# SamsungLabs/cloud_transformers

Measured on AMD Instinct MI355X. Metric: points/sec fwd+bwd MHCT, 4096-pt batch, 1/2/4/8 MI355X; % HBM roofline, higher is better.
Workload: dtype f32; 1 GPU; north-star op-level: B=8 clouds x N=4096 pts, H=64 heads, C=16 feat/head, 2D grid W=32, reduce=max, keys=tanh(randn), seed 1234+rank; step = Splat fwd, Slice fwd, Slice bwd, Splat bwd (key cotangents summed); per_gpu_batch=8, parallelism=replica-sharded clouds x1 (no collective), world_size_seen=1, hip_graph=True, steps_per_graph=10

## Files before the change

cloud_transformers_amd/_lib.py:

```python
import ctypes
import os
import subprocess
import threading

import torch

_HERE = os.path.dirname(os.path.abspath(__file__))
CSRC = os.path.join(_HERE, "csrc")
LIB_DIR = os.path.join(_HERE, "lib")
LIB_PATH = os.environ.get("CLOUDCT_LIB") or os.path.join(LIB_DIR, "libcloudct.so")
INCLUDE = os.path.join(os.path.dirname(_HERE), "include")

HIP_SOURCES = ["ct_raster.hip", "ct_mhct.hip", "ct_lattice.hip", "ct_gconv.hip", "ct_chamfer.hip", "ct_emd.hip",
               "ct_adain.hip", "ct_bnorm.hip", "ct_pwgemm.hip", "ct_nbr.hip", "ct_kpitems.hip", "ct_completion.hip", "ct_scanitems.hip",
               "ct_blockitems.hip", "ct_kpplan.hip", "ct_imageitems.hip", "ct_voxel.hip"]
HIPCC_FLAGS = ["-O3", "--offload-arch=gfx950", "-std=c++17", "-fPIC", "-shared",
               "-ffp-contract=off"]

class BnFwdItem(ctypes.Structure):
    _fields_ = [("x", ctypes.c_void_p), ("x_batch_stride", ctypes.c_longlong), ("weight", ctypes.c_void_p), ("bias", ctypes.c_void_p),
                ("running_mean", ctypes.c_void_p), ("running_var", ctypes.c_void_p), ("num_batches_tracked", ctypes.c_void_p),
                ("residual", ctypes.c_void_p), ("residual_batch_stride", ctypes.c_longlong), ("y", ctypes.c_void_p),
                ("y_batch_stride", ctypes.c_longlong), ("save_mean", ctypes.c_void_p), ("save_rstd", ctypes.c_void_p),
                ("amax_out", ctypes.c_void_p), ("C", ctypes.c_int), ("eps", ctypes.c_float), ("momentum", ctypes.c_float),
# ... 155 lines not shown
    deps = srcs + [os.path.join(INCLUDE, "cloudct_host.h")]
    if not force and os.path.exists(HOST_LIB_PATH) and all(os.path.getmtime(d) <= os.path.getmtime(HOST_LIB_PATH) for d in deps):
        return HOST_LIB_PATH
    import fcntl
    os.makedirs(LIB_DIR, exist_ok=True)
    with open(os.path.join(LIB_DIR, ".build_host.lock"), "w") as lock:
        fcntl.flock(lock, fcntl.LOCK_EX)
        try:
            tmp = "%s.%d.tmp" % (HOST_LIB_PATH, os.getpid())
            subprocess.run([os.environ.get("CXX", "g++"), "-O2", "-std=c++17", "-fPIC", "-shared", "-ffp-contract=off", "-I", INCLUDE]
                           + srcs + ["-o", tmp], check=True)
            os.replace(tmp, HOST_LIB_PATH)
        finally:
            fcntl.flock(lock, fcntl.LOCK_UN)
    return HOST_LIB_PATH


def load_host():
    global _host
    if _host is None:
        with _lock:
            if _host is None:
                lib = ctypes.CDLL(build_host())
                f32p, i32p = ctypes.POINTER(ctypes.c_float), ctypes.POINTER(ctypes.c_int32)
                lib.ct_grid_subsample.restype = ctypes.c_int64
                lib.ct_grid_subsample.argtypes = [f32p, f32p, i32p, ctypes.c_int64, ctypes.c_int, ctypes.c_int, ctypes.c_float,
                                                  f32p, f32p, i32p]
                _host = lib
    return _host


_vp, _i, _f, _sz = ctypes.c_void_p, ctypes.c_int, ctypes.c_float, ctypes.c_size_t
_ll = ctypes.c_longlong
_ip = ctypes.POINTER(ctypes.c_int)
_fp = ctypes.POINTER(ctypes.c_float)

SIGNATURES = {
    "ct_abi_version": (_i, []),
    "ct_strerror": (ctypes.c_char_p, [_i]),
    "ct_set_deterministic": (None, [_i]),
    "ct_get_deterministic": (_i, []),
    "ct_deterministic_override": (None, [_i]),
    "ct_positions_fwd": (_i, [_vp, _vp, _vp, _i, _i, _i, _i, _ip, _vp]),
    "ct_positions_bwd": (_i, [_vp, _vp, _vp, _i, _i, _i, _i, _ip, _vp]),
    "ct_splat_fwd": (_i, [_vp, _vp, _vp, _i, _vp, _i, _i, _i, _i, _i, _ip, _i, _vp]),
    "ct_splat_bwd_workspace_bytes": (_sz, [_i, _i, _i, _i, _i, _ip, _i]),
    "ct_splat_bwd": (_i, [_vp, _vp, _vp, _i, _vp, _vp, _vp, _vp, _vp, _sz, _i, _i, _i, _i, _i, _ip, _i, _vp]),
    "ct_splat_bwd_ex_workspace_bytes": (_sz, [_i, _i, _i, _i, _i, _ip, _i, _i]),
    "ct_splat_bwd_ex": (_i, [_vp, _vp, _vp, _i, _vp, _vp, _vp, _vp, _vp, _sz, _i, _i, _i, _i, _i, _ip, _i, _i, _vp]),
    "ct_debug_set_flags": (None, [ctypes.c_uint]),
    "ct_debug_set_nseg": (None, [_i]),
    "ct_debug_last_launch": (ctypes.c_char_p, []),
    "ct_slice_fwd": (_i, [_vp, _vp, _vp, _i, _vp, _i, _i, _i, _i, _i, _ip, _vp]),
    "ct_slice_bwd": (_i, [_vp, _vp, _vp, _i, _vp, _vp, _vp, _i, _i, _i, _i, _i, _ip, _vp]),
    "ct_slice_bwd_workspace_bytes": (_sz, [_i, _i, _i, _i, _i, _ip]),
    "ct_slice_bwd_ws": (_i, [_vp, _vp, _vp, _i, _vp, _vp, _vp, _vp, _sz, _i, _i, _i, _i, _i, _ip, _vp]),
    "ct_tickets_init": (_i, [_vp, _vp]),
    "ct_splat_bwd_tk_segments": (_i, [_i, _i, _i, _i, _i, _ip]),
    "ct_slice_bwd_tk": (_i, [_vp, _vp, _vp, _i, _vp, _vp, _vp, _vp, _sz, _vp, _i, _i, _i, _i, _i, _ip, _vp]),
    "ct_plane_sort_bytes": (_sz, [_i, _i, _i, _i, _ip]),
    "ct_plane_sort": (_i, [_vp, _vp, _sz, _i, _i, _i, _i, _ip, _vp]),
    "ct_slice_bwd_ps": (_i, [_vp, _vp, _vp, _i, _vp, _vp, _vp, _vp, _sz, _vp, _vp, _i, _i, _i, _i, _i, _ip, _vp]),
    "ct_splat_bwd_tk": (_i, [_vp, _vp, _vp, _i, _vp, _vp, _vp, _vp, _vp, _vp, _sz, _vp, _i, _i, _i, _i, _i, _ip, _i, _vp]),
    "ct_slice_bwd_grid": (_i, [_vp, _vp, _i, _vp, _vp, _i, _i, _i, _i, _i, _ip, _vp]),
    "ct_slice_bwd_keys": (_i, [_vp, _vp, _vp, _i, _vp, _vp, _i, _i, _i, _i, _i, _ip, _vp]),
    "ct_splat_lc_fwd": (_i, [_vp, _vp, _vp, _vp, _i, _vp, _i, _i, _i, _i, _i, _ip, _i, _vp]),
    "ct_splat_lc_bwd": (_i, [_vp, _vp, _vp, _vp, _i, _vp, _vp, _vp, _vp, _vp, _sz, _i, _i, _i, _i, _i, _ip, _i, _vp]),
    "ct_slice_lc_fwd": (_i, [_vp, _vp, _vp, _vp, _i, _vp, _i, _i, _i, _i, _i, _ip, _vp]),
    "ct_slice_lc_bwd": (_i, [_vp, _vp, _vp, _vp, _i, _vp, _vp, _vp, _i, _i, _i, _i, _i, _ip, _vp]),
    "ct_grid_occupancy": (_i, [_vp, ctypes.c_int64, _vp, _vp]),
    "ct_grid_occupancy_ratio": (_i, [_vp, ctypes.c_int64, _f, _vp, _vp, _vp]),
    "ct_lattice_fwd_workspace_bytes": (_sz, [_i, _i, _i]),
    "ct_lattice_fwd": (_i, [_vp, _vp, _vp, _vp, _vp, _vp, _vp, _vp, _vp, _vp, _sz, _i, _i, _i, _i, _vp]),
    "ct_lattice_bwd_workspace_bytes": (_sz, [_i, _i, _i]),
    "ct_lattice_bwd": (_i, [_vp] * 15 + [_vp, _sz, _i, _i, _i, _i, _vp]),
    "ct_lattice_so3_fwd": (_i, [_vp, _vp, _vp, _f, _vp, _vp, _vp, _vp, _vp, _vp, _vp, _vp, _sz, _vp, _i, _i, _i, _i, _vp]),
    "ct_lattice_so3_bwd": (_i, [_vp, _vp, _vp, _f] + [_vp] * 14 + [_vp, _sz, _i, _i, _i, _i, _vp]),
    "ct_so3_exp_fwd": (_i, [_vp, _vp, _i, _f, _vp]),
    "ct_so3_exp_bwd": (_i, [_vp, _vp, _vp, _i, _f, _vp]),
    "ct_adain_group_fwd": (_i, [_vp, _i, _i, _i, _vp]),
    "ct_adain_group_bwd": (_i, [_vp, _i, _i, _i, _vp]),
    "ct_bn_relu_supported": (_i, [_i, _i, _i]),
    "ct_bn_group_fwd": (_i, [_vp, _i, _i, _i, _vp]),
    "ct_bn_group_bwd": (_i, [_vp, _i, _i, _i, _vp]),
    "ct_bn_group_stats_fwd": (_i, [_vp, _i, _i, _i, _i, _i, _vp, _vp]),
    "ct_bn_group_apply_fwd": (_i, [_vp, _i, _i, _i, _i, _i, _vp, _i, _vp, _vp]),
    "ct_bn_group_reduce_bwd": (_i, [_vp, _i, _i, _i, _i, _i, _vp, _vp, _vp]),
    "ct_bn_group_apply_bwd": (_i, [_vp, _i, _i, _i, _i, _i, _vp, _vp, _vp]),
    "ct_bn_eval_supported": (_i, [_i, _i, _i]),
    "ct_bn_eval_group_fwd": (_i, [_vp, _i, _i, _i, _vp]),
    "ct_bn_eval_group_bwd": (_i, [_vp, _i, _i, _i, _vp]),
    "ct_gconv_fwd": (_i, [_vp, _vp, _vp, _vp, _i, _i, _i, _i, _i, _ip, _vp]),
    "ct_gconv_fwd_norm_supported": (_i, [_i, _i, _i, _i, _i, _ip]),
    "ct_gconv_fwd_norm": (_i, [_vp, _vp, _vp, _vp, _vp, _vp, _i, _vp, _i, _i, _i, _i, _i, _ip, _vp]),
    "ct_gconv_bwd_data": (_i, [_vp, _vp, _vp, _i, _i, _i, _i, _i, _ip, _vp]),
    "ct_gconv_supported": (_i, [_i, _i, _i, _i, _i, _ip]),
    "ct_set_gconv_precision": (None, [_i]),
    "ct_get_gconv_precision": (_i, []),
    "ct_gconv_precision_override": (None, [_i]),
    "ct_gconv_precision_covers": (_i, [_i, _i, _i, _i, _i, _i, _ip]),
    "ct_gconv_bwd_weight_workspace_bytes": (_sz, [_i, _i, _i, _i, _i, _ip]),
    "ct_gconv_bwd_weight": (_i, [_vp, _vp, _vp, _vp, _vp, _sz, _i, _i, _i, _i, _i, _ip, _vp]),
    "ct_mhct_core_supported": (_i, [_i, _i, _i, _i, _i, _ip]),
    "ct_mhct_core_workspace_bytes": (_sz, [_i, _i, _i, _i, _i, _ip]),
    "ct_mhct_core_workspace_init": (_i, [_vp, _sz, _i, _i, _i, _i, _i, _ip, _vp]),
    "ct_mhct_core_fwd": (_i, [_vp, _vp, _vp, _i, _vp, _vp, _vp, _vp, _vp, _vp, _vp, _sz, _i, _i, _i, _i, _i, _ip, _vp]),
# ... 104 lines not shown
```

cloud_transformers_amd/csrc/ct_raster.hip:

```cpp
#include "ct_common.h"
#include <string.h>
#include <type_traits>
#include <algorithm>
#include <atomic>
#include <mutex>

#ifndef CT_QUAD_THREADS
#define CT_QUAD_THREADS 512
#endif
#ifndef CT_QUAD_WAVES
#define CT_QUAD_WAVES 4
#endif
#ifndef CT_QUAD_CG
#define CT_QUAD_CG 4
#endif

namespace {

#include "ct_raster_args.h"

__device__ __forceinline__ float stats_MK(const RasterArgs& a, size_t bh, int ch, const float* tile, int G) {
  if (a.stats != nullptr) {
    const size_t per = (size_t)a.B * a.H * a.C;
    unsigned m = 0u, k = 0u;
// ... 933 lines not shown
          if (atomic) {
#pragma unroll
            for (int i = 0; i < 4; ++i) atomicAdd(pk + i, gs[i][j]);
          } else {
            float4 o = make_float4(gs[0][j], gs[1][j], gs[2][j], gs[3][j]);
            if (!first || a.accumulate) {
              const float4 prev = *(const float4*)pk;
              o.x += prev.x; o.y += prev.y; o.z += prev.z; o.w += prev.w;
            }
            *(float4*)pk = o;
          }
        }
      }
    }
    if (STATS) {
      __syncthreads();
      for (int ch = threadIdx.x; ch < cc; ch += blockDim.x) {
        unsigned m = 0u;
        for (int j = 0; j < 32; ++j) m = max(m, s_max[ch * 32 + j]);
        s_max[ch * 32] = m;
      }
      __syncthreads();
      unsigned kmax = 0;
      if (first) {
        for (int i = threadIdx.x; i <= a.cnt_mask; i += blockDim.x) kmax = max(kmax, (unsigned)s_cnt[i]);
        for (int o = 32; o > 0; o >>= 1) kmax = max(kmax, (unsigned)__shfl_xor((int)kmax, o, 64));
      }
      unsigned* slots = (unsigned*)(a.tile_out + toff);
      const bool split = a.nsplit > 1;
      unsigned* mine = a.stats != nullptr ? a.stats + ((size_t)sp * a.B * a.H * a.C + bh * a.C) * 2 : nullptr;
      if (first) {
        if ((threadIdx.x & 63) == 0) atomicMax((unsigned*)&s_cnt[0], kmax);
        __syncthreads();
        const unsigned kall = (unsigned)s_cnt[0];
        for (int ch = threadIdx.x; ch < a.C; ch += blockDim.x) {
          unsigned* kslot = (unsigned*)(a.tile_out + (bh * a.C + ch) * (size_t)g.G) + 1;
          if (mine != nullptr) mine[2 * ch + 1] = kall;
          else if (split) atomicAdd(kslot, kall);
          else *kslot = kall;
        }
      }
      for (int ch = threadIdx.x; ch < cc; ch += blockDim.x) {
        if (mine != nullptr) mine[2 * (c0 + ch)] = s_max[ch * 32];
        else if (split) atomicMax(slots + (size_t)ch * g.G, s_max[ch * 32]);
        else slots[(size_t)ch * g.G] = s_max[ch * 32];
      }
    }
    first = false;
  }
  if constexpr (NORM) norm_store_amax(am, lds, a.amax);
}

#include "ct_raster_hot.h"
#include "ct_raster_hot3d.h"
CT_KERNARG_IS_ARGS_AND_GRID((splat_max_bwd_hot_kernel<false, 32, 2>), 2);
CT_KERNARG_IS_ARGS_AND_GRID((splat_max_bwd_hot_kernel<true, 0, 0, kHotWideThreads>), 2);
#include "ct_raster_band.h"
#include "ct_raster_sorted.h"
#include "ct_raster_sorted3d.h"

template <int DIM>
__global__ void positions_fwd_kernel(const float* keys, float* lc, long long* idx, int BH, int N, GridW<DIM> g) {
  constexpr int V = 1 << DIM;
  size_t i = (size_t)blockIdx.x * blockDim.x + threadIdx.x;
  if (i >= (size_t)BH * N) return;
  size_t bh = i / N;
  int n = (int)(i % N);
  float w0[DIM], w1[DIM];
  int f[DIM];
#pragma unroll
  for (int j = 0; j < DIM; ++j) ct_axis(keys[(bh * DIM + j) * N + n], g.hw[j], g.W[j], w0[j], w1[j], f[j]);
  Corners<DIM> c;
  ct_corners<DIM>(w0, w1, f, g, c);
#pragma unroll
  for (int v = 0; v < V; ++v) {
    lc[(bh * V + v) * N + n] = c.w[v];
    idx[(bh * V + v) * N + n] = (long long)c.cell[v];
  }
}

template <int DIM>
__global__ void positions_bwd_kernel(const float* keys, const float* g_lc, float* g_keys, int BH, int N, GridW<DIM> g) {
  constexpr int V = 1 << DIM;
  size_t i = (size_t)blockIdx.x * blockDim.x + threadIdx.x;
  if (i >= (size_t)BH * N) return;
  size_t bh = i / N;
  int n = (int)(i % N);
  float w0[DIM], w1[DIM], mask[DIM], gw[V], gs[DIM];
  int f[DIM];
#pragma unroll
  for (int j = 0; j < DIM; ++j) {
    float k = keys[(bh * DIM + j) * N + n];
    ct_axis(k, g.hw[j], g.W[j], w0[j], w1[j], f[j]);
    mask[j] = ct_key_mask(k);
  }
#pragma unroll
  for (int v = 0; v < V; ++v) gw[v] = g_lc[(bh * V + v) * N + n];
  ct_corner_grad<DIM>(w0, w1, gw, gs);
#pragma unroll
  for (int j = 0; j < DIM; ++j) g_keys[(bh * DIM + j) * N + n] = gs[j] * mask[j];
}

__global__ void __launch_bounds__(1024) occupancy_kernel(const float* grid, long long n, unsigned long long* count) {
  __shared__ unsigned s_part[16];
  unsigned local = 0;
  const long long n4 = n >> 2;
// ... 48 lines not shown
    __hip_atomic_store(ws + 1 + blockIdx.x, t, __ATOMIC_RELAXED, __HIP_MEMORY_SCOPE_AGENT);
    asm volatile("s_waitcnt vmcnt(0)" ::: "memory");
    const unsigned old = __hip_atomic_fetch_add((unsigned*)ws, 1u, __ATOMIC_RELAXED, __HIP_MEMORY_SCOPE_AGENT);
    s_last = old == gridDim.x - 1u;
    if (old == gridDim.x - 1u) {
      __hip_atomic_store((unsigned*)ws, 0u, __ATOMIC_RELAXED, __HIP_MEMORY_SCOPE_AGENT);
      __builtin_amdgcn_fence(__ATOMIC_ACQUIRE, "agent");
      asm volatile("s_waitcnt vmcnt(0)" ::: "memory");
    }
  }
  __syncthreads();
  if (s_last) {
    unsigned long long t = 0;
    for (unsigned i = threadIdx.x; i < gridDim.x; i += blockDim.x)
      t += __hip_atomic_load(ws + 1 + i, __ATOMIC_RELAXED, __HIP_MEMORY_SCOPE_AGENT);
    unsigned lo = (unsigned)t;
    for (int off = 32; off > 0; off >>= 1) lo += __shfl_down(lo, off, 64);
    __syncthreads();
    if ((threadIdx.x & 63) == 0) s_part[threadIdx.x >> 6] = lo;
    __syncthreads();
    if (threadIdx.x == 0) {
      unsigned long long tot = 0;
      for (int w = 0; w < (int)(blockDim.x >> 6); ++w) tot += s_part[w];
      out[0] = (float)(long long)tot * inv;
    }
  }
}

__global__ void zero_slots_kernel(float* tiles, size_t stride, size_t rows) {
  const size_t r = (size_t)blockIdx.x * blockDim.x + threadIdx.x;
  if (r < rows) {
    tiles[r * stride] = 0.0f;
    tiles[r * stride + 1] = 0.0f;
  }
}

std::atomic<unsigned> t_dbg_flags{0};
std::atomic<int> t_dbg_nseg{0};
std::atomic<int> t_deterministic{0};
thread_local int t_det_override = -1;
inline bool det_now() { return t_det_override >= 0 ? t_det_override != 0 : t_deterministic.load(std::memory_order_relaxed) != 0; }
std::mutex t_last_mu;
char t_last[256] = "";

using ct_tags::note;
using ct_tags::note_reset;

struct Switches {
  unsigned flags;
  int nseg;
  int sorted;
  bool wide;
  bool det;
  bool has(unsigned f) const { return (flags & f) != 0; }
  bool hot() const { return !has(CT_DEBUG_NO_HOT); }
};
Switches read_switches() {
  static const auto env = [](const char* name, int unset) {
    const char* e = getenv(name);
    return e ? atoi(e) : unset;
  };
  static const int sorted = env("CLOUDCT_SORTED", -1), wide = env("CLOUDCT_WIDE", 1), nseg = env("CLOUDCT_SPLAT_BWD_NSEG", 0);
  const int dbg = t_dbg_nseg.load(std::memory_order_relaxed);
  return {t_dbg_flags.load(std::memory_order_relaxed), dbg ? dbg : nseg, sorted, wide != 0,
          det_now()};
}

struct Plan {
  int CC, nchunks, threads;
  size_t lds_bytes;
  bool lds_tile;
};

bool valid_common(int B, int H, int C, int N, int dim, const int* W) {
  if (B <= 0 || H <= 0 || C <= 0 || N <= 0 || (dim != 2 && dim != 3) || !W) return false;
  long long G = 1;
  for (int j = 0; j < dim; ++j) {
    if (W[j] < 2) return false;
    G *= W[j];
    if (G > (1ll << 30)) return false;
  }
  if (H > 65535 || B > 65535) return false;
  return true;
}

template <int DIM>
GridW<DIM> make_grid(const int* W) {
  GridW<DIM> g;
  g.G = 1;
  for (int j = 0; j < DIM; ++j) {
    g.W[j] = W[j];
    g.hw[j] = (float)(W[j] - 1) * 0.5f;
    g.G *= W[j];
  }
  return g;
}

int round_threads(int n) {
  int t = ((n + 63) / 64) * 64;
  return t < 64 ? 64 : (t > 1024 ? 1024 : t);
}

Plan make_plan(int B, int H, int C, int N, int G, int tiles_per_wg ,
               long long want = 256 , int min_cc = 4 ) {
  if (min_cc == 4 && (long long)B * H <= 64) min_cc = 1;
  Plan p;
  size_t per_ch = (size_t)G * 4 * tiles_per_wg;
  p.lds_tile = true;
  if (per_ch > (size_t)kBigLdsBytes) {
    p.lds_tile = false;
    p.CC = C;
    p.nchunks = 1;
    p.lds_bytes = 0;
    p.threads = round_threads(N);
    return p;
  }
  int cc_fit = (int)(kMaxLdsBytes / per_ch);
  if (cc_fit < min_cc) cc_fit = (int)((size_t)kBigLdsBytes / per_ch) < min_cc ? (int)((size_t)kBigLdsBytes / per_ch) : min_cc;
// ... 1020 lines not shown
  if (pg.lds_bytes + extra > (size_t)kBigLdsBytes) return CT_EINVAL;
  ga.cnt_mask = cnt - 1;
  ga.CC = pg.CC; ga.nchunks = pg.nchunks; ga.ncg = 1; ga.atomic_gpos = 0;
  ga.nsplit = slice_bwd_stats_nsplit(a.B, a.H, a.N);
  const size_t stats_bytes = (size_t)ga.nsplit * a.B * a.H * a.C * 2 * 4;
  unsigned* stats = nullptr;
  if (ga.nsplit > 1) {
    if (ws != nullptr && ws_bytes >= stats_bytes && ((uintptr_t)ws & 3) == 0) {
      stats = (unsigned*)ws;
    } else {
      const size_t rows = (size_t)a.B * a.H * a.C;
      CT_CLEAR_ERROR();
      hipLaunchKernelGGL(zero_slots_kernel, dim3((unsigned)((rows + 255) / 256)), dim3(256), 0, st, a.tile_out, (size_t)g.G, rows);
      CT_CHECK_LAUNCH();
    }
  }
  ga.stats = stats;
  dim3 ggrid(ga.nsplit, a.H, a.B);
  if (launch_quad<DIM, QM_GATHER_GW, (DIM == 2 ? CT_QUAD_CG : 2), CT_QUAD_THREADS, true>(ggrid, quad_threads(a.N, ga.nsplit), pg.lds_bytes + extra, st,
                                                                                         ga, g) != CT_OK)
    return CT_ELAUNCH;
  RasterArgs sa = a;
  sa.CC = ps.CC; sa.nchunks = ps.nchunks;
  sa.stats = stats; sa.nsplit = ga.nsplit;
  const int sthreads = ps.threads;
  dim3 sgrid(sa.nchunks, a.H, a.B);
  note(ga.nsplit > 1 ? (stats != nullptr ? "slice_bwd_gw_stats_parts" : "slice_bwd_gw_stats_nsplit") : "slice_bwd_gw_stats");
  if (scatter_quad_ok(sa, true, g.G)) {
    const int qt = scatter_quad_threads(DIM, a.N);
    if (sa.pad_dtype != CT_PAD_NONE) CT_LAUNCH((scatter_quad_kernel<DIM, true, true>), sgrid, qt, (size_t)sa.CC * g.G * 4 + (size_t)sa.CC * 8, st, sa, g);
    else CT_LAUNCH((scatter_quad_kernel<DIM, true, false>), sgrid, qt, (size_t)sa.CC * g.G * 4 + (size_t)sa.CC * 8, st, sa, g);
    note("scatter_quad_add");
    return CT_OK;
  }
  CT_LAUNCH((scatter_add_fx_stream_kernel<DIM, true>), sgrid, sthreads, (size_t)sa.CC * g.G * 4 + (size_t)2 * sa.CC * 4, st, sa, g);
  note("scatter_add_fx_stream");
  return CT_OK;
}

bool valid_pad(const void* pad, int pad_dtype) {
  if (pad_dtype == CT_PAD_NONE) return true;
  return (pad_dtype == CT_PAD_F32 || pad_dtype == CT_PAD_I32) && pad != nullptr;
}

RasterArgs base_args(int B, int H, int C, int N, const void* pad, int pad_dtype) {
  RasterArgs a = {};
  a.B = B; a.H = H; a.C = C; a.N = N;
  a.pad = pad_dtype == CT_PAD_NONE ? nullptr : pad;
  a.pad_dtype = pad_dtype;
  a.nsplit = 1; a.ncg = 1; a.nchunks = 1; a.CC = C;
  return a;
}

template <bool FROM_KEYS>
int splat_fwd_impl(PosSrc pos, const float* feat, const void* pad, int pad_dtype, float* grid,
                   int B, int H, int C, int N, int dim, const int* W, int reduce, hipStream_t st) {
  if (!valid_common(B, H, C, N, dim, W) || !feat || !grid || !valid_pad(pad, pad_dtype)) return CT_EINVAL;
  if (reduce != CT_REDUCE_MAX0 && reduce != CT_REDUCE_SUM) return CT_EINVAL;
  note_reset();
  const Switches sw = read_switches();
  RasterArgs a = base_args(B, H, C, N, pad, pad_dtype);
  a.pos = pos; a.src = feat; a.tile_out = grid;
  return dim == 2 ? run_scatter<2, FROM_KEYS>(sw, a, W, reduce == CT_REDUCE_SUM, st)
                  : run_scatter<3, FROM_KEYS>(sw, a, W, reduce == CT_REDUCE_SUM, st);
}

template <bool FROM_KEYS>
int splat_bwd_impl(PosSrc pos, const float* feat, const void* pad, int pad_dtype, const float* grid,
                   const float* g_grid, float* g_feat, float* g_pos, void* ws, size_t ws_bytes,
                   int B, int H, int C, int N, int dim, const int* W, int reduce, hipStream_t st,
                   const float* g_pos_add = nullptr, void* tickets = nullptr, const Switches* outer = nullptr) {
  if (!valid_common(B, H, C, N, dim, W) || !feat || !g_grid || !g_feat || !g_pos || !valid_pad(pad, pad_dtype)) return CT_EINVAL;
  note_reset();
  const Switches sw = outer ? *outer : read_switches();
  if (g_pos_add != nullptr) {
    const bool in_place = g_pos_add == g_pos;
    const size_t gpos_n = (size_t)B * H * (FROM_KEYS ? dim : (1 << dim)) * N;
    if (in_place && (!ws || ws_bytes < gpos_n * 4)) return CT_EWORKSPACE;
    const size_t head = in_place ? ws_bytes - gpos_n * 4 : ws_bytes;
    if (reduce == CT_REDUCE_MAX0 && grid) {
      RasterArgs a = base_args(B, H, C, N, pad, pad_dtype);
      a.pos = pos; a.src = feat; a.dst = g_feat; a.g_pos = g_pos; a.tile_in = grid; a.tile_in2 = g_grid;
      a.accumulate = in_place ? 1 : 0;
      a.gpos_add = g_pos_add;
      a.tickets = (unsigned*)tickets;
      const int r = dim == 2 ? run_splat_max_bwd<2, FROM_KEYS>(sw, a, W, ws, head, st) : run_splat_max_bwd<3, FROM_KEYS>(sw, a, W, ws, head, st);
      if (r != CT_EINVAL) return r;
    }
    if constexpr (FROM_KEYS) {
      if (reduce == CT_REDUCE_SUM && dim == 2) {
        RasterArgs a = base_args(B, H, C, N, pad, pad_dtype);
        a.pos = pos; a.src = feat; a.dst = g_feat; a.g_pos = g_pos; a.tile_in = g_grid;
        a.gpos_add = g_pos_add;
        const int r = run_splat_sum_bwd_hot(sw, a, make_grid<2>(W), st);
        if (r != CT_EINVAL) return r;
      }
    }
    float* tmp = in_place ? (float*)((char*)ws + head) : g_pos;
    const int r = splat_bwd_impl<FROM_KEYS>(pos, feat, pad, pad_dtype, grid, g_grid, g_feat, tmp, ws, head, B, H, C, N, dim, W,
                                            reduce, st, nullptr, tickets, &sw);
    if (r != CT_OK) return r;
    CT_CLEAR_ERROR();
    hipLaunchKernelGGL(add_inplace_kernel, dim3((unsigned)((gpos_n + 255) / 256)), dim3(256), 0, st, g_pos,
                       in_place ? (const float*)tmp : g_pos_add, gpos_n);
    CT_CHECK_LAUNCH();
    note("add_inplace");
// ... 143 lines not shown
  if (!valid_common(B, H, C, N, dim, W) || reduce != CT_REDUCE_MAX0) return 0;
  size_t n = splat_bwd_workspace_generic(B, H, C, N, dim, W);
  if (det_now()) {
    size_t G = 1;
    for (int j = 0; j < dim; ++j) G *= W[j];
    n = std::max(n, splat_bwd_det_plan(B, H, C, N, dim, (int)G).workspace());
  }
  const size_t hot = dim == 2 ? splat_bwd_hot_workspace(B, H, C, N, make_grid<2>(W)) : splat_bwd_hot_workspace(B, H, C, N, make_grid<3>(W));
  return std::max(n, hot);
}

int ct_splat_bwd(const float* keys, const float* feat, const void* pad, int pad_dtype, const float* grid,
                 const float* g_grid, float* g_feat, float* g_keys, void* ws, size_t ws_bytes,
                 int B, int H, int C, int N, int dim, const int* W, int reduce, ct_stream_t s) {
  if (!keys) return CT_EINVAL;
  PosSrc pos = {keys, nullptr, nullptr};
  return splat_bwd_impl<true>(pos, feat, pad, pad_dtype, grid, g_grid, g_feat, g_keys, ws, ws_bytes,
                              B, H, C, N, dim, W, reduce, (hipStream_t)s);
}

size_t ct_splat_bwd_ex_workspace_bytes(int B, int H, int C, int N, int dim, const int* W, int reduce, int flags) {
  size_t n = ct_splat_bwd_workspace_bytes(B, H, C, N, dim, W, reduce);
  if ((flags & CT_BWD_ACCUMULATE_KEYS) && valid_common(B, H, C, N, dim, W)) n += (size_t)B * H * dim * N * 4;
  return n;
}

int ct_splat_bwd_ex(const float* keys, const float* feat, const void* pad, int pad_dtype, const float* grid,
                    const float* g_grid, float* g_feat, float* g_keys, void* ws, size_t ws_bytes,
                    int B, int H, int C, int N, int dim, const int* W, int reduce, int flags, ct_stream_t s) {
  if (!keys || (flags & ~CT_BWD_ACCUMULATE_KEYS)) return CT_EINVAL;
  PosSrc pos = {keys, nullptr, nullptr};
  return splat_bwd_impl<true>(pos, feat, pad, pad_dtype, grid, g_grid, g_feat, g_keys, ws, ws_bytes,
                              B, H, C, N, dim, W, reduce, (hipStream_t)s, (flags & CT_BWD_ACCUMULATE_KEYS) ? g_keys : nullptr);
}

void ct_debug_set_flags(unsigned flags) { t_dbg_flags = flags; }

void ct_set_deterministic(int on) { t_deterministic.store(on ? 1 : 0, std::memory_order_relaxed); }
int ct_get_deterministic(void) { return det_now() ? 1 : 0; }
void ct_deterministic_override(int on) { t_det_override = on < 0 ? -1 : (on ? 1 : 0); }

const char* ct_debug_last_launch(void) {
  static thread_local char copy[256];
  std::lock_guard<std::mutex> lk(t_last_mu);
  memcpy(copy, t_last, sizeof(copy));
  return copy;
}

int ct_slice_fwd(const float* keys, const float* grid, const void* pad, int pad_dtype, float* out,
                 int B, int H, int C, int N, int dim, const int* W, ct_stream_t s) {
  if (!keys) return CT_EINVAL;
  PosSrc pos = {keys, nullptr, nullptr};
  return slice_fwd_impl<true>(pos, grid, pad, pad_dtype, out, B, H, C, N, dim, W, (hipStream_t)s);
}

int ct_slice_bwd(const float* keys, const float* grid, const void* pad, int pad_dtype, const float* g_out,
                 float* g_grid, float* g_keys, int B, int H, int C, int N, int dim, const int* W, ct_stream_t s) {
  if (!keys) return CT_EINVAL;
  PosSrc pos = {keys, nullptr, nullptr};
  return slice_bwd_impl<true>(pos, grid, pad, pad_dtype, g_out, g_grid, g_keys, B, H, C, N, dim, W, (hipStream_t)s);
}

size_t ct_slice_bwd_workspace_bytes(int B, int H, int C, int N, int dim, const int* W) {
  if (!valid_common(B, H, C, N, dim, W)) return 0;
  const Switches sw = read_switches();
  const size_t hot = dim == 2 ? slice_bwd_hot_workspace(sw, B, H, C, N, make_grid<2>(W)) : slice_bwd_hot_workspace(sw, B, H, C, N, make_grid<3>(W));
  const int ns = slice_bwd_stats_nsplit(B, H, N);
  const size_t stats = ns > 1 ? (size_t)ns * B * H * C * 8 : 0;
  return hot > stats ? hot : stats;
}

int ct_slice_bwd_ws(const float* keys, const float* grid, const void* pad, int pad_dtype, const float* g_out,
                    float* g_grid, float* g_keys, void* ws, size_t ws_bytes, int B, int H, int C, int N, int dim,
                    const int* W, ct_stream_t s) {
  if (!keys) return CT_EINVAL;
  PosSrc pos = {keys, nullptr, nullptr};
  return slice_bwd_impl<true>(pos, grid, pad, pad_dtype, g_out, g_grid, g_keys, B, H, C, N, dim, W, (hipStream_t)s, ws, ws_bytes);
}

void ct_debug_set_nseg(int nseg) { t_dbg_nseg.store(nseg, std::memory_order_relaxed); }

int ct_splat_bwd_tk_segments(int B, int H, int C, int N, int dim, const int* W) {
  if (!valid_common(B, H, C, N, dim, W)) return 1;
  const Switches sw = read_switches();
  long long G = 1;
  for (int j = 0; j < dim; ++j) G *= W[j];
  if (!hot_shape_ok(sw, B, H, C, N, (int)G, 0) || (long long)B * H > CT_TICKETS_BYTES / 8) return 1;
  if (sw.det && !sw.has(CT_DEBUG_FORCE_BAND)) return 1;
  if (sw.has(CT_DEBUG_FORCE_BAND) && C == 4 && ((G / W[0]) & 3) == 0 && W[0] >= 4) return 2;
  HotPlan sp;
  const int nseg = splat_bwd_segments_plan(sw, B, H, C, N, (int)G, dim, sp);
  if (nseg == 0) {
    return (C == 4 && ((G / W[0]) & 3) == 0 && W[0] >= 4 && (size_t)G * 4 > (size_t)kBigLdsBytes && !sw.has(CT_DEBUG_NO_BAND)) ? 2 : 1;
  }
  return nseg;
}

int ct_tickets_init(void* tickets, ct_stream_t s) {
  if (!tickets || ((uintptr_t)tickets & 3) != 0) return CT_EINVAL;
  return hipMemsetAsync(tickets, 0, CT_TICKETS_BYTES, (hipStream_t)s) == hipSuccess ? CT_OK : CT_ELAUNCH;
}

int ct_slice_bwd_tk(const float* keys, const float* grid, const void* pad, int pad_dtype, const float* g_out,
                    float* g_grid, float* g_keys, void* ws, size_t ws_bytes, void* tickets, int B, int H, int C, int N, int dim,
                    const int* W, ct_stream_t s) {
  if (!keys) return CT_EINVAL;
// ... 158 lines not shown
```

cloud_transformers_amd/step.py:

```python
import torch

from . import _lib
from . import determinism as _det
from .ops import _ptr, _stream, sizes_of


class SplatSliceStep:

    def __init__(self, keys, feat, cot, tensor_size, heads, dim, reduce="max", tickets=True, plane_sort=False):
        assert keys.is_cuda and feat.is_cuda and cot.is_cuda
        self.W = sizes_of(tensor_size, dim)
        self.H, self.dim, self.reduce = heads, dim, reduce
        self.B, HC, self.N = feat.shape
        self.C = HC // heads
        self.keys, self.feat, self.cot = keys.contiguous(), feat.contiguous(), cot.contiguous()
        dev = feat.device
        self.z = torch.empty(self.B, HC, *self.W, device=dev)
        self.out = torch.empty_like(self.feat)
        self.g_z = torch.empty_like(self.z)
        self.g_feat = torch.empty_like(self.feat)
        self.g_keys_buf = torch.empty_like(self.keys)
        self.g_keys_out = self.g_keys_buf
        self.lib = _lib.load()
        self.deterministic = _det.push(self.lib)
        self.Wa = _lib.int_array(self.W)
        self.red = _lib.REDUCE[reduce]
        nws = self.lib.ct_splat_bwd_ex_workspace_bytes(self.B, self.H, self.C, self.N, dim, self.Wa, self.red,
                                                       _lib.BWD_ACCUMULATE_KEYS)
        self.ws = torch.empty(nws, device=dev, dtype=torch.uint8) if nws else None
        self.nws = nws
        nws2 = self.lib.ct_slice_bwd_workspace_bytes(self.B, self.H, self.C, self.N, dim, self.Wa)
        self.ws2 = torch.empty(nws2, device=dev, dtype=torch.uint8) if nws2 else None
        self.nws2 = nws2
        self.tickets = torch.zeros(_lib.TICKETS_BYTES // 4, device=dev, dtype=torch.int32) if tickets else None
        nps = self.lib.ct_plane_sort_bytes(self.B, self.H, self.N, dim, self.Wa) if plane_sort else 0
        self.sorted = torch.empty(nps, device=dev, dtype=torch.uint8) if nps else None
        self.nps = nps
        if tickets and reduce == "max" and self.lib.ct_splat_bwd_tk_segments(self.B, self.H, self.C, self.N, dim, self.Wa) > 1:
            self.g_keys_out = torch.empty_like(self.keys)

    def plane_sort(self):
        if self.sorted is not None:
            _lib.check(self.lib.ct_plane_sort(_ptr(self.keys), _ptr(self.sorted), self.nps, self.B, self.H, self.N, self.dim,
                                              self.Wa, _stream()), "ct_plane_sort")

    def splat_fwd(self):
        _lib.check(self.lib.ct_splat_fwd(_ptr(self.keys), _ptr(self.feat), None, 0, _ptr(self.z),
                                         self.B, self.H, self.C, self.N, self.dim, self.Wa, self.red, _stream()),
                   "ct_splat_fwd")

    def slice_fwd(self):
        _lib.check(self.lib.ct_slice_fwd(_ptr(self.keys), _ptr(self.z), None, 0, _ptr(self.out),
                                         self.B, self.H, self.C, self.N, self.dim, self.Wa, _stream()),
                   "ct_slice_fwd")

    def slice_bwd_grid(self):
        _lib.check(self.lib.ct_slice_bwd_grid(_ptr(self.keys), None, 0, _ptr(self.cot), _ptr(self.g_z),
                                              self.B, self.H, self.C, self.N, self.dim, self.Wa, _stream()),
                   "ct_slice_bwd_grid")

    def slice_bwd_keys(self):
        _lib.check(self.lib.ct_slice_bwd_keys(_ptr(self.keys), _ptr(self.z), None, 0, _ptr(self.cot),
                                              _ptr(self.g_keys_buf),
                                              self.B, self.H, self.C, self.N, self.dim, self.Wa, _stream()),
                   "ct_slice_bwd_keys")

    def slice_bwd(self):
        _lib.check(self.lib.ct_slice_bwd_ps(_ptr(self.keys), _ptr(self.z), None, 0, _ptr(self.cot),
                                            _ptr(self.g_z), _ptr(self.g_keys_buf), _ptr(self.ws2), self.nws2, _ptr(self.tickets),
                                            _ptr(self.sorted), self.B, self.H, self.C, self.N, self.dim, self.Wa, _stream()),
                   "ct_slice_bwd_ps")

    def splat_bwd(self):
        _lib.check(self.lib.ct_splat_bwd_tk(_ptr(self.keys), _ptr(self.feat), None, 0, _ptr(self.z), _ptr(self.g_z),
                                            _ptr(self.g_feat), _ptr(self.g_keys_buf), _ptr(self.g_keys_out), _ptr(self.ws), self.nws,
                                            _ptr(self.tickets), self.B, self.H, self.C, self.N, self.dim, self.Wa, self.red,
                                            _stream()),
                   "ct_splat_bwd_tk")

    PASSES = ("splat_fwd", "slice_fwd", "slice_bwd", "splat_bwd")

    KERNEL_OF = {
        "scatter_quad_max": "scatter_quad_kernel<2, false, false, 32>",
        "scatter_add_fx_reg": "scatter_add_fx_reg_kernel",
        "scatter_add_fused": "slice_bwd_fused_kernel<false, 32, 2, false>",
        "scatter_add_sorted": "slice_bwd_sorted_kernel<false, 32, false, false",
        "splat_sum_bwd_hot": "splat_sum_bwd_kernel",
        "gather_ci": "gather_ci_kernel",
        "gather_quad": "quad_kernel<2, 0,",
        "slice_bwd_fused": "slice_bwd_fused_kernel",
        "slice_bwd_sorted": "slice_bwd_sorted_kernel<false, 32, false, true",
        "slice_bwd_presorted": "slice_bwd_sorted_kernel<false, 32, true, true",
        "splat_max_bwd_hot": "splat_max_bwd_hot_kernel",
        "splat_max_bwd_whole_head": "quad_kernel<2, 2, 4, 1024,",
    }

    HEADLINE_KERNELS = {
        "splat_fwd": "scatter_quad_kernel<2, false, false, 32>",
        "slice_fwd": "gather_ci_kernel<false, 32>",
        "slice_bwd": "slice_bwd_sorted_kernel<false, 32, false, true, 4096, 16>",
        "splat_bwd": "splat_max_bwd_hot_kernel<false, 32, 2, 512>",
    }

    def launch_tags(self):
        tags = {}
        for name in self.PASSES:
            getattr(self, name)()
            tags[name] = self.lib.ct_debug_last_launch().decode()
        return tags

    def run(self):
        self.lib.ct_set_deterministic(1 if self.deterministic else 0)
        self.plane_sort()
        self.splat_fwd()
        self.slice_fwd()
        self.slice_bwd()
        self.splat_bwd()

    def g_keys(self):
        return self.g_keys_out

    def algorithmic_bytes(self):
        P = self.B * self.N * self.H
        G = 1
        for w in self.W:
            G *= w
        kb = 4 * self.dim * P
        fb = 4 * self.C * P
        gb = 4 * self.C * G * self.B * self.H
        per = {
            "splat_fwd": kb + fb + gb,
            "slice_fwd": kb + gb + fb,
            "slice_bwd": kb + fb + gb + gb + kb,
            "splat_bwd": kb + fb + gb + gb + fb + kb,
        }
        per["total"] = sum(per.values())
        return per
```

include/cloudct.h:

```cpp
#ifndef CLOUDCT_H
#define CLOUDCT_H

#include <stddef.h>
#include <stdint.h>

#ifdef __cplusplus
extern "C" {
#endif

#define CT_ABI_VERSION 3

#define CT_OK 0
#define CT_EINVAL (-1)
#define CT_ELAUNCH (-2)
#define CT_EWORKSPACE (-3)
#define CT_EPRECOND (-4)

#define CT_REDUCE_MAX0 0
#define CT_REDUCE_SUM 1

#define CT_PAD_NONE 0
#define CT_PAD_F32 1
#define CT_PAD_I32 2

typedef void* ct_stream_t;

int ct_abi_version(void);
const char* ct_strerror(int status);

void ct_set_deterministic(int on);
int ct_get_deterministic(void);
void ct_deterministic_override(int on);

int ct_positions_fwd(const float* keys, float* local_coord, int64_t* flat_idx,
                     int B, int H, int N, int dim, const int* W, ct_stream_t s);
int ct_positions_bwd(const float* keys, const float* g_local_coord, float* g_keys,
                     int B, int H, int N, int dim, const int* W, ct_stream_t s);

int ct_splat_fwd(const float* keys, const float* feat, const void* pad, int pad_dtype,
                 float* grid, int B, int H, int C, int N, int dim, const int* W,
                 int reduce, ct_stream_t s);
size_t ct_splat_bwd_workspace_bytes(int B, int H, int C, int N, int dim, const int* W, int reduce);
int ct_splat_bwd(const float* keys, const float* feat, const void* pad, int pad_dtype,
                 const float* grid, const float* g_grid, float* g_feat, float* g_keys,
                 void* workspace, size_t workspace_bytes,
                 int B, int H, int C, int N, int dim, const int* W, int reduce, ct_stream_t s);

#define CT_BWD_ACCUMULATE_KEYS 1
size_t ct_splat_bwd_ex_workspace_bytes(int B, int H, int C, int N, int dim, const int* W, int reduce, int flags);
int ct_splat_bwd_ex(const float* keys, const float* feat, const void* pad, int pad_dtype,
                    const float* grid, const float* g_grid, float* g_feat, float* g_keys,
                    void* workspace, size_t workspace_bytes,
                    int B, int H, int C, int N, int dim, const int* W, int reduce, int flags, ct_stream_t s);

#define CT_DEBUG_NO_HOT 1
#define CT_DEBUG_FORCE_HOT 2
#define CT_DEBUG_NO_BAND 4
#define CT_DEBUG_FORCE_BAND 8
#define CT_DEBUG_NO_SORTED 16
#define CT_DEBUG_FORCE_SORTED 32
#define CT_DEBUG_FORCE_SORTED_SEG 64
#define CT_DEBUG_NO_WIDE 128
void ct_debug_set_flags(unsigned flags);
const char* ct_debug_last_launch(void);
void ct_debug_set_nseg(int nseg);

int ct_slice_fwd(const float* keys, const float* grid, const void* pad, int pad_dtype,
                 float* out, int B, int H, int C, int N, int dim, const int* W, ct_stream_t s);
int ct_slice_bwd(const float* keys, const float* grid, const void* pad, int pad_dtype,
                 const float* g_out, float* g_grid, float* g_keys,
                 int B, int H, int C, int N, int dim, const int* W, ct_stream_t s);
size_t ct_slice_bwd_workspace_bytes(int B, int H, int C, int N, int dim, const int* W);
int ct_slice_bwd_ws(const float* keys, const float* grid, const void* pad, int pad_dtype,
                    const float* g_out, float* g_grid, float* g_keys, void* workspace, size_t workspace_bytes,
                    int B, int H, int C, int N, int dim, const int* W, ct_stream_t s);
#define CT_TICKETS_BYTES 65536
int ct_tickets_init(void* tickets, ct_stream_t s);
int ct_slice_bwd_tk(const float* keys, const float* grid, const void* pad, int pad_dtype,
                    const float* g_out, float* g_grid, float* g_keys, void* workspace, size_t workspace_bytes,
                    void* tickets, int B, int H, int C, int N, int dim, const int* W, ct_stream_t s);
size_t ct_plane_sort_bytes(int B, int H, int N, int dim, const int* W);
int ct_plane_sort(const float* keys, void* sorted, size_t sorted_bytes, int B, int H, int N, int dim, const int* W, ct_stream_t s);
int ct_slice_bwd_ps(const float* keys, const float* grid, const void* pad, int pad_dtype,
                    const float* g_out, float* g_grid, float* g_keys, void* workspace, size_t workspace_bytes,
                    void* tickets, const void* sorted, int B, int H, int C, int N, int dim, const int* W, ct_stream_t s);
int ct_splat_bwd_tk_segments(int B, int H, int C, int N, int dim, const int* W);
int ct_splat_bwd_tk(const float* keys, const float* feat, const void* pad, int pad_dtype,
                    const float* grid, const float* g_grid, float* g_feat, const float* g_keys_add, float* g_keys,
                    void* workspace, size_t workspace_bytes, void* tickets,
                    int B, int H, int C, int N, int dim, const int* W, int reduce, ct_stream_t s);
int ct_slice_bwd_grid(const float* keys, const void* pad, int pad_dtype, const float* g_out,
                      float* g_grid, int B, int H, int C, int N, int dim, const int* W, ct_stream_t s);
int ct_slice_bwd_keys(const float* keys, const float* grid, const void* pad, int pad_dtype,
                      const float* g_out, float* g_keys,
                      int B, int H, int C, int N, int dim, const int* W, ct_stream_t s);

int ct_splat_lc_fwd(const float* local_coord, const int64_t* flat_idx, const float* feat,
                    const void* pad, int pad_dtype, float* grid,
                    int B, int H, int C, int N, int dim, const int* W, int reduce, ct_stream_t s);
int ct_splat_lc_bwd(const float* local_coord, const int64_t* flat_idx, const float* feat,
                    const void* pad, int pad_dtype, const float* grid, const float* g_grid,
                    float* g_feat, float* g_local_coord, void* workspace, size_t workspace_bytes,
                    int B, int H, int C, int N, int dim, const int* W, int reduce, ct_stream_t s);
int ct_slice_lc_fwd(const float* local_coord, const int64_t* flat_idx, const float* grid,
                    const void* pad, int pad_dtype, float* out,
                    int B, int H, int C, int N, int dim, const int* W, ct_stream_t s);
int ct_slice_lc_bwd(const float* local_coord, const int64_t* flat_idx, const float* grid,
                    const void* pad, int pad_dtype, const float* g_out,
                    float* g_grid, float* g_local_coord,
                    int B, int H, int C, int N, int dim, const int* W, ct_stream_t s);

int ct_grid_occupancy(const float* grid, int64_t n_elements, int64_t* count, ct_stream_t s);
#define CT_OCC_WORKSPACE_BYTES 4096
int ct_grid_occupancy_ratio(const float* grid, int64_t n_elements, float inv_denominator, float* out, void* workspace, ct_stream_t s);

size_t ct_lattice_fwd_workspace_bytes(int B, int H, int N);
int ct_lattice_fwd(const float* xyz, const float* residual, const float* R, const float* shift,
                   const float* scales, const float* kscale, float* keys, float* lattice,
                   float* key_stats ,
                   void* workspace, size_t workspace_bytes, int B, int H, int N, int dim, ct_stream_t s);
size_t ct_lattice_bwd_workspace_bytes(int B, int H, int N);
int ct_lattice_bwd(const float* xyz, const float* residual, const float* R, const float* shift,
                   const float* scales, const float* kscale, const float* lattice, const float* g_lattice,
                   const float* g_keys, float* g_xyz, float* g_residual, float* g_R, float* g_shift, float* g_scales,
// ... 238 lines not shown
```

Baseline: 188.5 million points/s.

## Fuse splat and slice forward into one kernel keeping the grid in LDS

Adds a fused 2D max-splat plus slice forward kernel. Each block splats its points into an LDS grid tile, writes the tile to global memory for backward, transposes it in LDS, and immediately slices from LDS. This avoids re-reading the grid and keys from HBM and saves a launch. The cost is a large LDS footprint and 1024-thread blocks, which may limit occupancy. It is enabled by default only for the B*H>=512, W=32, C=16, N=4096 shape.

```diff
diff --git a/cloud_transformers_amd/_lib.py b/cloud_transformers_amd/_lib.py
--- a/cloud_transformers_amd/_lib.py
+++ b/cloud_transformers_amd/_lib.py
@@ -231,6 +231,8 @@
     "ct_debug_set_nseg": (None, [_i]),
     "ct_debug_last_launch": (ctypes.c_char_p, []),
     "ct_slice_fwd": (_i, [_vp, _vp, _vp, _i, _vp, _i, _i, _i, _i, _i, _ip, _vp]),
+    "ct_splat_slice_fwd_supported": (_i, [_i, _i, _i, _i, _i, _ip, _i, _i]),
+    "ct_splat_slice_fwd": (_i, [_vp, _vp, _vp, _i, _vp, _vp, _i, _i, _i, _i, _i, _ip, _i, _vp]),
     "ct_slice_bwd": (_i, [_vp, _vp, _vp, _i, _vp, _vp, _vp, _i, _i, _i, _i, _i, _ip, _vp]),
     "ct_slice_bwd_workspace_bytes": (_sz, [_i, _i, _i, _i, _i, _ip]),
     "ct_slice_bwd_ws": (_i, [_vp, _vp, _vp, _i, _vp, _vp, _vp, _vp, _sz, _i, _i, _i, _i, _i, _ip, _vp]),
diff --git a/cloud_transformers_amd/csrc/ct_raster.hip b/cloud_transformers_amd/csrc/ct_raster.hip
--- a/cloud_transformers_amd/csrc/ct_raster.hip
+++ b/cloud_transformers_amd/csrc/ct_raster.hip
@@ -1009,6 +1009,7 @@
 }
 
 #include "ct_raster_hot.h"
+#include "ct_raster_fwd_fused.h"
 #include "ct_raster_hot3d.h"
 CT_KERNARG_IS_ARGS_AND_GRID((splat_max_bwd_hot_kernel<false, 32, 2>), 2);
 CT_KERNARG_IS_ARGS_AND_GRID((splat_max_bwd_hot_kernel<true, 0, 0, kHotWideThreads>), 2);
@@ -1163,6 +1164,8 @@
   int sorted;
   bool wide;
   bool det;
+  int fused_fwd;
+  int fused_geom;
   bool has(unsigned f) const { return (flags & f) != 0; }
   bool hot() const { return !has(CT_DEBUG_NO_HOT); }
 };
@@ -1172,9 +1175,10 @@
     return e ? atoi(e) : unset;
   };
   static const int sorted = env("CLOUDCT_SORTED", -1), wide = env("CLOUDCT_WIDE", 1), nseg = env("CLOUDCT_SPLAT_BWD_NSEG", 0);
+  static const int fused_fwd = env("CLOUDCT_FUSED_FWD", -1), fused_geom = env("CLOUDCT_FUSED_FWD_GEOM", 0);
   const int dbg = t_dbg_nseg.load(std::memory_order_relaxed);
   return {t_dbg_flags.load(std::memory_order_relaxed), dbg ? dbg : nseg, sorted, wide != 0,
-          det_now()};
+          det_now(), fused_fwd, fused_geom};
 }
 
 struct Plan {
@@ -2301,6 +2305,58 @@
   return a;
 }
 
+constexpr const char* kFusedFwdTag = "splat_slice_fwd_fused";
+enum FusedFwdGeom { kFusedGeomPlane = 1, kFusedGeomChunk8 = 2 };
+constexpr FusedFwdGeom kFusedFwdDefaultGeom = kFusedGeomChunk8;
+constexpr bool kFusedFwdMeasuredWin = true;
+struct FusedFwdPlan {
+  bool ok;
+  FusedFwdGeom geom;
+  int CC, nchunks, threads;
+  size_t lds;
+};
+
+FusedFwdPlan fused_fwd_plan(const Switches sw, int B, int H, int C, int N, int dim, const int* W, int reduce, int pad_dtype,
+                            uintptr_t ptr_bits) {
+  FusedFwdPlan p = {};
+  if (!valid_common(B, H, C, N, dim, W) || dim != 2 || reduce != CT_REDUCE_MAX0 || !sw.hot()) return p;
+  if (pad_dtype != CT_PAD_NONE && pad_dtype != CT_PAD_F32 && pad_dtype != CT_PAD_I32) return p;
+  const int G = W[0] * W[1];
+  if ((N & 3) != 0 || (N >> 2) > kFusedFwdThreads || (C & 3) != 0 || (G & 3) != 0 || (ptr_bits & 15) != 0) return p;
+  p.geom = sw.fused_geom == kFusedGeomPlane ? kFusedGeomPlane : sw.fused_geom == kFusedGeomChunk8 ? kFusedGeomChunk8 : kFusedFwdDefaultGeom;
+  p.CC = p.geom == kFusedGeomPlane ? C : std::min(C, 8);
+  p.nchunks = (C + p.CC - 1) / p.CC;
+  p.lds = (size_t)2 * p.CC * G * 4;
+  if (p.lds > (size_t)(p.geom == kFusedGeomPlane ? kBigLdsBytes : kHalfCuLdsBytes)) return p;
+  p.threads = round_threads(N >> 2);
+  const bool measured = kFusedFwdMeasuredWin && (long long)B * H >= 512 && W[0] == 32 && W[1] == 32 && C == 16 && N == 4096 &&
+                        pad_dtype == CT_PAD_NONE;
+  p.ok = measured || sw.has(CT_DEBUG_FORCE_HOT) || sw.fused_fwd == 1;
+  return p;
+}
+
+int run_splat_slice_fwd(const FusedFwdPlan& p, RasterArgs a, const int* W, hipStream_t st) {
+  const GridW<2> g = make_grid<2>(W);
+  a.CC = p.CC;
+  a.nchunks = p.nchunks;
+  const dim3 grid(p.nchunks, a.H, a.B);
+  const int r = with_pad_extent<true, 32>(a, g, [&](auto pad, auto wt) {
+    constexpr bool PAD = decltype(pad)::value;
+    constexpr int WT = decltype(wt)::value;
+    if constexpr (WT == 32) {
+      if (p.geom == kFusedGeomChunk8) {
+        CT_LAUNCH((splat_slice_fwd_kernel<PAD, WT, 8>), grid, p.threads, p.lds, st, a, g);
+        return CT_OK;
+      }
+    }
+    CT_LAUNCH((splat_slice_fwd_kernel<PAD, WT, 4>), grid, p.threads, p.lds, st, a, g);
+    return CT_OK;
+  });
+  if (r != CT_OK) return r;
+  note(kFusedFwdTag);
+  return CT_OK;
+}
+
 template <bool FROM_KEYS>
 int splat_fwd_impl(PosSrc pos, const float* feat, const void* pad, int pad_dtype, float* grid,
                    int B, int H, int C, int N, int dim, const int* W, int reduce, hipStream_t st) {
@@ -2550,6 +2606,24 @@
   if (!keys) return CT_EINVAL;
   PosSrc pos = {keys, nullptr, nullptr};
   return slice_fwd_impl<true>(pos, grid, pad, pad_dtype, out, B, H, C, N, dim, W, (hipStream_t)s);
+}
+
+int ct_splat_slice_fwd_supported(int B, int H, int C, int N, int dim, const int* W, int reduce, int pad_dtype) {
+  return fused_fwd_plan(read_switches(), B, H, C, N, dim, W, reduce, pad_dtype, 0).ok ? 1 : 0;
+}
+
+int ct_splat_slice_fwd(const float* keys, const float* feat, const void* pad, int pad_dtype, float* grid, float* out,
+                       int B, int H, int C, int N, int dim, const int* W, int reduce, ct_stream_t s) {
+  if (!keys || !feat || !grid || !out || !valid_pad(pad, pad_dtype)) return CT_EINVAL;
+  const Switches sw = read_switches();
+  const uintptr_t bits = (uintptr_t)keys | (uintptr_t)feat | (uintptr_t)grid | (uintptr_t)out;
+  const FusedFwdPlan p = fused_fwd_plan(sw, B, H, C, N, dim, W, reduce, pad_dtype, bits);
+  if (!p.ok) return CT_EINVAL;
+  note_reset();
+  RasterArgs a = base_args(B, H, C, N, pad, pad_dtype);
+  a.pos = {keys, nullptr, nullptr};
+  a.src = feat; a.tile_out = grid; a.dst = out;
+  return run_splat_slice_fwd(p, a, W, (hipStream_t)s);
 }
 
 int ct_slice_bwd(const float* keys, const float* grid, const void* pad, int pad_dtype, const float* g_out,
diff --git a/cloud_transformers_amd/csrc/ct_raster_fwd_fused.h b/cloud_transformers_amd/csrc/ct_raster_fwd_fused.h
--- /dev/null
+++ b/cloud_transformers_amd/csrc/ct_raster_fwd_fused.h
@@ -0,0 +1,135 @@
+#pragma once
+
+constexpr int kFusedFwdThreads = 1024;
+
+template <bool HAS_PAD, int WT, int MINW>
+__global__ void __launch_bounds__(kFusedFwdThreads, MINW) splat_slice_fwd_kernel(RasterArgs a, GridW<2> g_arg) {
+  const GridW<2> g = grid2_of<WT>(g_arg);
+  extern __shared__ __align__(16) float lds[];
+  const int G = WT ? WT * WT : g.G, W1 = WT ? WT : g.W[1], N = a.N;
+  unsigned* acc = (unsigned*)lds;
+  float4* T4 = (float4*)(lds + (size_t)a.CC * G);
+  const BlockXHB blk = block_xhb();
+  const int chunk = blk.x, h = blk.h, b = blk.b;
+  const size_t bh = (size_t)b * a.H + h;
+  const int c0 = chunk * a.CC;
+  const int cc = min(a.CC, a.C - c0);
+  const int tid = threadIdx.x, nq = N >> 2;
+  const bool mine = tid < nq;
+  const int n0 = min(tid, nq - 1) << 2;
+  const int off[4] = {0, W1, 1, W1 + 1};
+
+  const float4 tx = *(const float4*)(a.pos.keys + (bh * 2 + 0) * N + n0);
+  const float4 ty = *(const float4*)(a.pos.keys + (bh * 2 + 1) * N + n0);
+  for (int i = tid; i < (cc * G) >> 2; i += blockDim.x) ((int4*)acc)[i] = make_int4(0, 0, 0, 0);
+  constexpr bool HOLD = MINW <= 4;
+  const float kx[4] = {tx.x, tx.y, tx.z, tx.w}, ky[4] = {ty.x, ty.y, ty.z, ty.w};
+  float cw[4][4], pv[4];
+  int base[4];
+  {
+#pragma unroll
+    for (int i = 0; i < 4; ++i) {
+      Pt2 p;
+      pt2_from_keys(kx[i], ky[i], g, W1, p);
+      base[i] = p.base;
+#pragma unroll
+      for (int v = 0; v < 4; ++v) cw[i][v] = p.cw[v];
+      pv[i] = HAS_PAD ? ct_load_pad(a.pad, a.pad_dtype, (size_t)b * N + n0 + i) : 1.0f;
+    }
+  }
+  __syncthreads();
+
+  if (mine) {
+    const float* src = a.src + (bh * a.C + c0) * (size_t)N + n0;
+    for (int cg0 = 0; cg0 < cc; cg0 += 4) {
+      float fv[4][4];
+#pragma unroll
+      for (int cj = 0; cj < 4; ++cj) {
+        const float4 t = *(const float4*)(src + (size_t)(cg0 + cj) * N);
+        fv[cj][0] = t.x; fv[cj][1] = t.y; fv[cj][2] = t.z; fv[cj][3] = t.w;
+      }
+#pragma unroll
+      for (int cj = 0; cj < 4; ++cj) {
+        unsigned* Tc = acc + (size_t)(cg0 + cj) * G;
+#pragma unroll
+        for (int i = 0; i < 4; ++i) {
+          const float f = HAS_PAD ? fv[cj][i] * pv[i] : fv[cj][i];
+#pragma unroll
+          for (int v = 0; v < 4; ++v) {
+            const float prod = f * cw[i][v];
+            if (prod > 0.0f) atomicMax(Tc + base[i] + off[v], __float_as_uint(prod));
+          }
+        }
+      }
+    }
+  }
+  __syncthreads();
+
+  {
+    const int G4 = G >> 2, n = (cc >> 2) * G4;
+    float* zout = a.tile_out + (bh * a.C + c0) * (size_t)G;
+    for (int j = tid; j < n; j += blockDim.x) {
+      const int q = j / G4, cell = (j - q * G4) << 2;
+      const size_t row = (size_t)(q * 4) * G + cell;
+      float4 r[4];
+#pragma unroll
+      for (int k = 0; k < 4; ++k) r[k] = *(const float4*)(lds + row + (size_t)k * G);
+#pragma unroll
+      for (int k = 0; k < 4; ++k) *(float4*)(zout + row + (size_t)k * G) = r[k];
+      float4* d = T4 + ((size_t)j << 2);
+      d[0] = make_float4(r[0].x, r[1].x, r[2].x, r[3].x);
+      d[1] = make_float4(r[0].y, r[1].y, r[2].y, r[3].y);
+      d[2] = make_float4(r[0].z, r[1].z, r[2].z, r[3].z);
+      d[3] = make_float4(r[0].w, r[1].w, r[2].w, r[3].w);
+    }
+  }
+  __syncthreads();
+
+  if (mine) {
+    float* drow = a.dst + (bh * a.C + c0) * (size_t)N + n0;
+    const float4* Tq = T4;
+    for (int cq = 0; cq < (cc >> 2); ++cq, Tq += G) {
+      float o[4][4];
+#pragma unroll
+      for (int i = 0; i < 4; ++i) {
+        float w[4];
+        int bi;
+        if constexpr (HOLD) {
+          bi = base[i];
+#pragma unroll
+          for (int v = 0; v < 4; ++v) w[v] = cw[i][v];
+        } else {
+          float kxi = kx[i], kyi = ky[i];
+          asm volatile("" : "+v"(kxi), "+v"(kyi));
+          __builtin_amdgcn_sched_barrier(0);
+          Pt2 p;
+          pt2_from_keys(kxi, kyi, g, W1, p);
+          bi = p.base;
+#pragma unroll
+          for (int v = 0; v < 4; ++v) w[v] = p.cw[v];
+        }
+        float4 cv[4];
+#pragma unroll
+        for (int v = 0; v < 4; ++v) cv[v] = Tq[bi + off[v]];
+        float s0 = cv[0].x * w[0], s1 = cv[0].y * w[0], s2 = cv[0].z * w[0], s3 = cv[0].w * w[0];
+#pragma unroll
+        for (int v = 1; v < 4; ++v) {
+          s0 += cv[v].x * w[v];
+          s1 += cv[v].y * w[v];
+          s2 += cv[v].z * w[v];
+          s3 += cv[v].w * w[v];
+        }
+        o[0][i] = HAS_PAD ? s0 * pv[i] : s0;
+        o[1][i] = HAS_PAD ? s1 * pv[i] : s1;
+        o[2][i] = HAS_PAD ? s2 * pv[i] : s2;
+        o[3][i] = HAS_PAD ? s3 * pv[i] : s3;
+        if constexpr (!HOLD) {
+          asm volatile("" : "+v"(o[0][i]), "+v"(o[1][i]), "+v"(o[2][i]), "+v"(o[3][i]));
+          __builtin_amdgcn_sched_barrier(0);
+        }
+      }
+#pragma unroll
+      for (int cj = 0; cj < 4; ++cj, drow += N) st_stream4(drow, make_float4(o[cj][0], o[cj][1], o[cj][2], o[cj][3]));
+    }
+  }
+}
diff --git a/cloud_transformers_amd/step.py b/cloud_transformers_amd/step.py
--- a/cloud_transformers_amd/step.py
+++ b/cloud_transformers_amd/step.py
@@ -1,3 +1,5 @@
+import os
+
 import torch
 
 from . import _lib
@@ -36,6 +38,9 @@
         nps = self.lib.ct_plane_sort_bytes(self.B, self.H, self.N, dim, self.Wa) if plane_sort else 0
         self.sorted = torch.empty(nps, device=dev, dtype=torch.uint8) if nps else None
         self.nps = nps
+        self.fused_fwd = (os.environ.get("CLOUDCT_FUSED_FWD", "") != "0" and
+                          bool(self.lib.ct_splat_slice_fwd_supported(self.B, self.H, self.C, self.N, dim, self.Wa, self.red, 0)))
+        self._forward_tag = None
         if tickets and reduce == "max" and self.lib.ct_splat_bwd_tk_segments(self.B, self.H, self.C, self.N, dim, self.Wa) > 1:
             self.g_keys_out = torch.empty_like(self.keys)
 
@@ -53,6 +58,11 @@
         _lib.check(self.lib.ct_slice_fwd(_ptr(self.keys), _ptr(self.z), None, 0, _ptr(self.out),
                                          self.B, self.H, self.C, self.N, self.dim, self.Wa, _stream()),
                    "ct_slice_fwd")
+
+    def splat_slice_fwd(self):
+        _lib.check(self.lib.ct_splat_slice_fwd(_ptr(self.keys), _ptr(self.feat), None, 0, _ptr(self.z), _ptr(self.out),
+                                               self.B, self.H, self.C, self.N, self.dim, self.Wa, self.red, _stream()),
+                   "ct_splat_slice_fwd")
 
     def slice_bwd_grid(self):
         _lib.check(self.lib.ct_slice_bwd_grid(_ptr(self.keys), None, 0, _ptr(self.cot), _ptr(self.g_z),
@@ -87,6 +97,7 @@
         "scatter_add_sorted": "slice_bwd_sorted_kernel<false, 32, false, false",
         "splat_sum_bwd_hot": "splat_sum_bwd_kernel",
         "gather_ci": "gather_ci_kernel",
+        "splat_slice_fwd_fused": "splat_slice_fwd_kernel",
         "gather_quad": "quad_kernel<2, 0,",
         "slice_bwd_fused": "slice_bwd_fused_kernel",
         "slice_bwd_sorted": "slice_bwd_sorted_kernel<false, 32, false, true",
@@ -112,10 +123,22 @@
     def run(self):
         self.lib.ct_set_deterministic(1 if self.deterministic else 0)
         self.plane_sort()
-        self.splat_fwd()
-        self.slice_fwd()
+        self.forward()
         self.slice_bwd()
         self.splat_bwd()
+
+    def forward(self):
+        record = self._forward_tag is None
+        tags = []
+        for call in ((self.splat_slice_fwd,) if self.fused_fwd else (self.splat_fwd, self.slice_fwd)):
+            call()
+            if record:
+                tags.append(self.lib.ct_debug_last_launch().decode())
+        if record:
+            self._forward_tag = "+".join(tags)
+
+    def forward_tag(self):
+        return self._forward_tag
 
     def g_keys(self):
         return self.g_keys_out
diff --git a/include/cloudct.h b/include/cloudct.h
--- a/include/cloudct.h
+++ b/include/cloudct.h
@@ -70,6 +70,10 @@
 int ct_slice_bwd(const float* keys, const float* grid, const void* pad, int pad_dtype,
                  const float* g_out, float* g_grid, float* g_keys,
                  int B, int H, int C, int N, int dim, const int* W, ct_stream_t s);
+int ct_splat_slice_fwd_supported(int B, int H, int C, int N, int dim, const int* W, int reduce, int pad_dtype);
+int ct_splat_slice_fwd(const float* keys, const float* feat, const void* pad, int pad_dtype,
+                       float* grid, float* out, int B, int H, int C, int N, int dim, const int* W,
+                       int reduce, ct_stream_t s);
 size_t ct_slice_bwd_workspace_bytes(int B, int H, int C, int N, int dim, const int* W);
 int ct_slice_bwd_ws(const float* keys, const float* grid, const void* pad, int pad_dtype,
                     const float* g_out, float* g_grid, float* g_keys, void* workspace, size_t workspace_bytes,
```

After: 192.7 million points/s, median of 6. 1.02x the previous value.
